# stevesuyao/KinectDepthMapEnhancement

Hardware: AMD Instinct MI355X
Metric: Mpixels/sec joint-bilateral filtered (640x480 & 1080p); % HBM roofline (higher is better)
Workload: dtype f32; 1 GPU; JointBilateralFilter::Process (K0 pre-smooth 5/30/30 + K1) on 64 x 640x480 synthetic RGB-D frames (64 per GPU), window 11 (radius 5), sigma_s 3 px, sigma_r 7.65/255, sigma_d 20 mm; frames_per_gpu=64, width=640, height=480, window=11, kernel_variant=auto (w11-pk2-16x16-false-v4)

## Files before the change

kinectdepthmapenhancement_amd/csrc/jbf_fast.hip:

```cpp
#include "kde_internal.h"
#include "kde_device_math.h"

#include <type_traits>

namespace kde {
namespace {

constexpr uint32_t kMagic = 0x4B000000u;
constexpr uint32_t kOff = 1u << 18;
constexpr uint32_t kInvalidBias = 0xFF000000u;
constexpr float kBiasF = 8388608.0f + 262144.0f;
constexpr uint32_t kNegHBits = 0xCB7C0000u;
constexpr double kScaleLog2 = 24.0;

struct FastArgs {
    const float* depth;
    const uint8_t* guide;
    float* out;
    int width, height, n;
    int tiles_x, tiles_y;
    FastDiv24 div_tiles, div_tx;
    float kc;
    float sd;
    float t_skip;
    float t2_skip;
    int cd_skip;
    int vec4;
    KDE_STAGE(float* stage_avg; unsigned* stage_counters; int stage_force;)
    const float* tab_dev;
    __attribute__((aligned(8))) float tab[882];
};

__device__ __forceinline__ uint32_t dot4(uint32_t a, uint32_t b, uint32_t c)
{
    return __builtin_amdgcn_udot4(a, b, c, false);
}


template <int WIN, int PX, int BX, int BY, bool CACHE, bool CSKIP>
__global__ __launch_bounds__(BX* BY) void jbf_fast_kernel(const FastArgs a)
{
    constexpr int R = WIN / 2;
    constexpr int NT = BX * BY;
    constexpr int TW = BX * PX, TH = BY;
    constexpr int LW = TW + 2 * R, LH = TH + 2 * R;
    constexpr int P = LW;
    constexpr int SEG = PX + 2 * R;
    __shared__ float s_d[LH * P];
    __shared__ uint32_t s_c[LH * P];
    __shared__ uint32_t s_n[LH * P];

    const unsigned nblk = gridDim.x;
    const unsigned lin = blockIdx.x;
    const unsigned per = nblk / 8, rem = nblk % 8;
    const unsigned xcd = lin % 8, slot = lin / 8;
    const unsigned id = xcd * per + (xcd < rem ? xcd : rem) + slot;
    const unsigned tiles = (unsigned)a.tiles_x * a.tiles_y;
    const unsigned frame_i = fastdiv24(id, a.div_tiles);
    const unsigned tile = id - frame_i * tiles;
    const int tyi = (int)fastdiv24(tile, a.div_tx), txi = tile - tyi * a.tiles_x;
    const int x0 = txi * TW, y0 = tyi * TH;

    const size_t frame = (size_t)frame_i * a.width * a.height;
    const float* __restrict__ depth = a.depth + frame;
    const uint8_t* __restrict__ guide = a.guide + frame * 3;
    const int tid = threadIdx.x;

    for (int i = tid; i < LW * LH; i += NT) {
        const int ly = i / LW, lx = i - ly * LW;
        const int gx = x0 + lx - R, gy = y0 + ly - R;
        float d = 0.0f;
        uint32_t c = 0;
        if (gx >= 0 && gx < a.width && gy >= 0 && gy < a.height) {
            const size_t q = (size_t)gy * a.width + gx;
            d = depth[q];
            const uint8_t* p = guide + q * 3;
            c = (uint32_t)p[0] | ((uint32_t)p[1] << 8) | ((uint32_t)p[2] << 16);
        }
        const bool valid = d > 50.0f;
        s_d[ly * P + lx] = valid ? d : 0.0f;
        s_c[ly * P + lx] = c;
        s_n[ly * P + lx] = valid ? (kMagic + kOff) - dot4(c, c, 0) : kInvalidBias;
    }
    __syncthreads();

    const int tx = tid % BX, ty = tid / BX;
    const int xb = x0 + tx * PX, y = y0 + ty;
    if (xb >= a.width || y >= a.height) return;

    uint32_t cc[PX];
    float cA[PX], skipA[PX];
    uint32_t thrU[PX];
#pragma unroll
    for (int k = 0; k < PX; k++) {
        cc[k] = s_c[(ty + R) * P + tx * PX + R + k];
        const uint32_t na = dot4(cc[k], cc[k], 0);
        cA[k] = -a.kc * (kBiasF + (float)na);
        skipA[k] = __builtin_fmaf(kBiasF + (float)na, a.kc, cA[k]);
        thrU[k] = CSKIP ? (kMagic + kOff) + na - (uint32_t)a.cd_skip : 0;
    }

    float arg[CACHE ? WIN * WIN * PX : 1];
    float wsum[PX], wgt[PX];
#pragma unroll
    for (int k = 0; k < PX; k++) wsum[k] = wgt[k] = 0.0f;

    auto arg1_of = [&](uint32_t cq, uint32_t nq, int k, float ls) -> float {
        const uint32_t u = (dot4(cq, cc[k], 0) << 1) + nq;
        float a1 = __builtin_fmaf(__uint_as_float(u), a.kc, cA[k]);
        if (CSKIP) a1 = (u <= thrU[k]) ? skipA[k] : a1;
        return a1 + ls;
    };

    auto pass1_row = [&](int i) {
        float dr[SEG];
        uint32_t cr[SEG], nr[SEG];
        const int rb = (ty + i) * P + tx * PX;
#pragma unroll
        for (int q = 0; q < SEG; q++) {
            dr[q] = s_d[rb + q];
            cr[q] = s_c[rb + q];
            nr[q] = s_n[rb + q];
        }
#pragma unroll
        for (int j = 0; j < WIN; j++) {
            const float ls = a.tab[i * WIN + j];
#pragma unroll
            for (int k = 0; k < PX; k++) {
                const float a1 = arg1_of(cr[j + k], nr[j + k], k, ls);
                if (CACHE) arg[(i * WIN + j) * PX + k] = a1;
                const float f = __builtin_amdgcn_exp2f(a1);
                wsum[k] = __builtin_fmaf(dr[j + k], f, wsum[k]);
                wgt[k] += f;
            }
        }
    };
    if (CACHE) {
#pragma unroll
        for (int i = 0; i < WIN; i++) pass1_row(i);
    } else {
#pragma unroll 1
        for (int i = 0; i < WIN; i++) pass1_row(i);
    }

    float c2[PX], num[PX], den[PX];
#pragma unroll
    for (int k = 0; k < PX; k++) {
        c2[k] = wsum[k] / wgt[k];
        num[k] = den[k] = 0.0f;
    }

    auto pass2_row = [&](int i) {
        float dr[SEG];
        uint32_t cr[SEG], nr[SEG];
        const int rb = (ty + i) * P + tx * PX;
#pragma unroll
        for (int q = 0; q < SEG; q++) {
            dr[q] = s_d[rb + q];
            if (!CACHE) {
                cr[q] = s_c[rb + q];
                nr[q] = s_n[rb + q];
            }
        }
#pragma unroll
        for (int j = 0; j < WIN; j++) {
            const float ls = CACHE ? 0.0f : a.tab[i * WIN + j];
#pragma unroll
            for (int k = 0; k < PX; k++) {
                const float a1 = CACHE ? arg[(i * WIN + j) * PX + k] : arg1_of(cr[j + k], nr[j + k], k, ls);
                const float t = (dr[j + k] - c2[k]) * a.sd;
                float a2 = __builtin_fmaf(-t, t, a1);
                a2 = (__builtin_fabsf(t) >= a.t_skip) ? a1 : a2;
                const float f = __builtin_amdgcn_exp2f(a2);
                num[k] = __builtin_fmaf(dr[j + k], f, num[k]);
                den[k] += f;
            }
        }
    };
    if (CACHE) {
#pragma unroll
        for (int i = 0; i < WIN; i++) pass2_row(i);
    } else {
#pragma unroll 1
        for (int i = 0; i < WIN; i++) pass2_row(i);
    }

    float* __restrict__ o = a.out + frame + (size_t)y * a.width + xb;
#pragma unroll
    for (int k = 0; k < PX; k++) {
        float r = 0.0f;
        if (wgt[k] > 0.0f) r = (den[k] == 0.0f) ? 0.0f : num[k] / den[k];
        if (xb + k < a.width) o[k] = r;
        KDE_STAGE(if (a.stage_avg && xb + k < a.width) a.stage_avg[frame + (size_t)y * a.width + xb + k] = c2[k];)
    }
}


typedef float f2 __attribute__((ext_vector_type(2)));
typedef uint32_t u2 __attribute__((ext_vector_type(2)));

__device__ __forceinline__ f2 pk_fma(f2 a, f2 b, f2 c) { return __builtin_elementwise_fma(a, b, c); }
__device__ __forceinline__ f2 bcast(float v) { return f2{v, v}; }
__device__ __forceinline__ f2 pk_add_clamp(f2 a, f2 b)
{
    f2 r;
    asm("v_pk_add_f32 %0, %1, %2 clamp" : "=v"(r) : "v"(a), "v"(b));
    return r;
}
__device__ __forceinline__ f2 pk_mul_clamp(f2 a, f2 b)
{
    f2 r;
    asm("v_pk_mul_f32 %0, %1, %2 clamp" : "=v"(r) : "v"(a), "v"(b));
    return r;
}

constexpr int pk_min_waves(int win, int np, bool cache, bool cskip, bool elide_on)
{
    if (win >= 23) return 3;
    if (win == 5 && np == 1 && cache) return 5;
    return 1;
}

template <int WIN, int NP, int BX, int BY, bool CACHE, bool CSKIP, bool VL, bool ELIDE_ON = true, int CR = (CACHE ? WIN : 0)>
__global__ __launch_bounds__(BX* BY) __attribute__((amdgpu_waves_per_eu(pk_min_waves(WIN, NP, CACHE, CSKIP, ELIDE_ON))))
void jbf_pk_kernel(const FastArgs a)
{
    static_assert(CR == (CACHE ? WIN : 0), "cached rows: all or none");
    constexpr int R = WIN / 2;
    constexpr int PX = 2 * NP;
    constexpr int NT = BX * BY;
    constexpr int TW = BX * PX, TH = BY;
    constexpr int LH = TH + 2 * R;
    constexpr int S1 = 0;
    constexpr int RA = !VL ? R : ((R + 3) / 4 * 4);
    constexpr int SH = VL ? ((RA - R) & 1) : 0;
    constexpr bool ALIGNED = ((RA - R + SH) % 2) == 0;
    constexpr int G = (RA + TW + R + 3) / 4;
    constexpr int P = VL ? (SH + 4 * G + 1) / 2 * 2 : (TW + 2 * R);
    constexpr int SEGP = NP + R;
    constexpr int HALF = (WIN - 1) / 2;
    static_assert(RA >= R && P % 2 == 0 && (!VL || ((RA + S1) % 4 == 0 && TW % 4 == 0 && (SH != 0 || P % 4 == 0))), "tile geometry");
    __shared__ __attribute__((aligned(16))) float s_d[LH * P];
    __shared__ __attribute__((aligned(16))) uint32_t s_c[LH * P];
    __shared__ __attribute__((aligned(16))) float s_n[LH * P];

    const unsigned nblk = gridDim.x;
    const unsigned lin = blockIdx.x;
    const unsigned per = nblk / 8, rem = nblk % 8;
    const unsigned xcd = lin % 8, slot = lin / 8;
    const unsigned id = xcd * per + (xcd < rem ? xcd : rem) + slot;
    const unsigned tiles = (unsigned)a.tiles_x * a.tiles_y;
    const unsigned frame_i = fastdiv24(id, a.div_tiles);
    const unsigned tile = id - frame_i * tiles;
    const int tyi = (int)fastdiv24(tile, a.div_tx), txi = tile - tyi * a.tiles_x;
    const int x0 = txi * TW - S1, y0 = tyi * TH;
    const int o = x0 - RA;

    const size_t frame = (size_t)frame_i * a.width * a.height;
    const float* __restrict__ depth = a.depth + frame;
    const uint8_t* __restrict__ guide = a.guide + frame * 3;
    const int tid = threadIdx.x;

    constexpr bool ELIDE = WIN >= 9 && ELIDE_ON;
    __shared__ uint32_t s_stat[8];
    if (ELIDE) {
        if (tid < 8) s_stat[tid] = (tid == 0 || (tid >= 2 && !(tid & 1))) ? 0xffffffffu : 0u;
        __syncthreads();
    }
    uint32_t st_dmin = 0x7f800000u, st_dmax = 0u, st_cmin[3] = {255u, 255u, 255u}, st_cmax[3] = {0u, 0u, 0u};
    auto stat = [&](float dv, uint32_t c, bool inside) {
        if (!ELIDE) return;
        if (dv > 0.0f) {
            st_dmin = min(st_dmin, __float_as_uint(dv));
            st_dmax = max(st_dmax, __float_as_uint(dv));
        }
        if (inside) {
#pragma unroll
            for (int ch = 0; ch < 3; ch++) {
                const uint32_t v = (c >> (8 * ch)) & 0xffu;
                st_cmin[ch] = min(st_cmin[ch], v);
                st_cmax[ch] = max(st_cmax[ch], v);
            }
        }
    };

    if (!VL) {
        for (int i = tid; i < P * LH; i += NT) {
            const int ly = i / P, lx = i - ly * P;
            const int gx = o + lx, gy = y0 - R + ly;
            float d = 0.0f;
            uint32_t c = 0;
            const bool inside = gx >= 0 && gx < a.width && gy >= 0 && gy < a.height;
            if (inside) {
                const size_t q = (size_t)gy * a.width + gx;
                d = depth[q];
                const uint8_t* p = guide + q * 3;
                c = (uint32_t)p[0] | ((uint32_t)p[1] << 8) | ((uint32_t)p[2] << 16);
            }
            const bool valid = d > 50.0f;
            s_d[i] = valid ? d : 0.0f;
            s_c[i] = c;
            s_n[i] = __uint_as_float(dot4(c, c, kNegHBits));
            stat(valid ? d : 0.0f, c, inside);
        }
    }
    for (int g = tid; VL && g < G * LH; g += NT) {
        const int ly = g / G, gi = g - ly * G;
        const int gx = o + 4 * gi, gy = y0 - R + ly;
        float d[4] = {0.0f, 0.0f, 0.0f, 0.0f};
        uint32_t c[4] = {0u, 0u, 0u, 0u};
        if (gy >= 0 && gy < a.height) {
            const size_t q = (size_t)gy * a.width + gx;
            if (a.vec4 && gx >= 0 && gx + 3 < a.width) {
                const float4 dv = *reinterpret_cast<const float4*>(depth + q);
                const uint32_t* cp = reinterpret_cast<const uint32_t*>(guide + q * 3);
                const uint32_t w0 = cp[0], w1 = cp[1], w2 = cp[2];
                d[0] = dv.x; d[1] = dv.y; d[2] = dv.z; d[3] = dv.w;
                c[0] = w0 & 0xffffffu;
                c[1] = (w0 >> 24) | ((w1 & 0xffffu) << 8);
                c[2] = (w1 >> 16) | ((w2 & 0xffu) << 16);
                c[3] = w2 >> 8;
            } else {
#pragma unroll
                for (int k = 0; k < 4; k++) {
                    if (gx + k >= 0 && gx + k < a.width) {
                        d[k] = depth[q + k];
                        const uint8_t* p = guide + (q + k) * 3;
                        c[k] = (uint32_t)p[0] | ((uint32_t)p[1] << 8) | ((uint32_t)p[2] << 16);
                    }
                }
            }
        }
        float nn[4];
#pragma unroll
        for (int k = 0; k < 4; k++) {
            const bool valid = d[k] > 50.0f;
            d[k] = valid ? d[k] : 0.0f;
            nn[k] = __uint_as_float(dot4(c[k], c[k], kNegHBits));
            stat(d[k], c[k], gy >= 0 && gy < a.height && gx + k >= 0 && gx + k < a.width);
        }
        const int li = ly * P + 4 * gi + SH;
        if constexpr (SH == 0) {
            *reinterpret_cast<float4*>(&s_d[li]) = make_float4(d[0], d[1], d[2], d[3]);
            *reinterpret_cast<uint4*>(&s_c[li]) = make_uint4(c[0], c[1], c[2], c[3]);
            *reinterpret_cast<float4*>(&s_n[li]) = make_float4(nn[0], nn[1], nn[2], nn[3]);
        } else {
#pragma unroll
            for (int k = 0; k < 4; k++) {
                s_d[li + k] = d[k];
                s_c[li + k] = c[k];
                s_n[li + k] = nn[k];
            }
        }
    }
    if (ELIDE) {
        uint32_t v[8] = {st_dmin, st_dmax, st_cmin[0], st_cmax[0], st_cmin[1], st_cmax[1], st_cmin[2], st_cmax[2]};
#pragma unroll
        for (int k = 0; k < 8; k++) {
#pragma unroll
            for (int m = 32; m >= 1; m >>= 1) {
                const uint32_t ov = (uint32_t)__shfl_xor((int)v[k], m, 64);
                v[k] = (k & 1) ? max(v[k], ov) : min(v[k], ov);
            }
        }
        if ((tid & 63) == 0) {
#pragma unroll
            for (int k = 0; k < 8; k++) {
                if (k & 1) atomicMax(&s_stat[k], v[k]);
                else atomicMin(&s_stat[k], v[k]);
            }
        }
    }
    __syncthreads();

    bool tile_c = CSKIP, tile_d = true;
    if (ELIDE) {
        const int rb = (int)s_stat[3] - (int)s_stat[2], rg = (int)s_stat[5] - (int)s_stat[4], rr = (int)s_stat[7] - (int)s_stat[6];
        if (s_stat[3] >= s_stat[2]) tile_c = CSKIP && (rb * rb + rg * rg + rr * rr >= a.cd_skip);
        const float range = __uint_as_float(s_stat[1]) - __uint_as_float(s_stat[0]);
        const float slack = __uint_as_float(s_stat[1]) * (float)(WIN * WIN + 8) * 0x1p-24f;
        tile_d = !((range * 1.0001f + slack) * a.sd < a.t_skip);
    }
    KDE_STAGE(if (a.stage_force) { tile_c = CSKIP; tile_d = true; })
    KDE_STAGE(if (a.stage_counters && tid == 0) {
        int body;
        if constexpr (!ELIDE) body = (CSKIP ? 1 : 0) + 2;
        else if constexpr (WIN >= 15) body = ((CSKIP && tile_c) || tile_d) ? (CSKIP ? 1 : 0) + 2 : 0;
        else body = ((CSKIP && tile_c) ? 1 : 0) + (tile_d ? 2 : 0);
        atomicAdd(&a.stage_counters[body], 1u);
    })

    const int tx = tid % BX, ty = tid / BX;
    const int xb = x0 + tx * PX, y = y0 + ty;
    if (xb >= a.width || y >= a.height) return;
    const int sx = SH + RA - R + tx * PX;

    uint32_t cc[PX];
    f2 negC[NP];
#pragma unroll
    for (int pp = 0; pp < NP; pp++) {
#pragma unroll
        for (int h = 0; h < 2; h++) {
            const int k = 2 * pp + h;
            cc[k] = s_c[(ty + R) * P + sx + R + k];
            const uint32_t na = dot4(cc[k], cc[k], 0);
            negC[pp][h] = -((float)kOff + (float)na);
        }
    }

    f2 kc2 = bcast(a.kc);
    asm volatile("" : "+v"(kc2));
    f2 arg[CR > 0 ? CR * WIN * NP : 1];
    f2 wsum[NP], wgt[NP];
#pragma unroll
    for (int pp = 0; pp < NP; pp++) wsum[pp] = wgt[pp] = bcast(0.0f);

    const f2 Tc = bcast((float)a.cd_skip);
    const f2 T2 = bcast(a.t2_skip);
    const f2 kBig = bcast(0x1p100f);

    auto unit_arg = [&](auto cs_tag, const u2* cp, const f2* np, int pp, int i, int u) -> f2 {
        constexpr bool CS = decltype(cs_tag)::value;
        uint32_t c0, c1;
        f2 hq;
        if (u <= HALF) {
            c0 = cp[pp + u].x; c1 = cp[pp + u].y; hq = np[pp + u];
        } else if (u < WIN - 1) {
            const int m = pp + (u - HALF);
            c0 = cp[m].y; c1 = cp[m].x; hq = __builtin_shufflevector(np[m], np[m], 1, 0);
        } else {
            c0 = cp[pp].y; c1 = cp[pp + HALF].x; hq = bcast(0.0f);
        }
        const f2 ab = f2{__uint_as_float(dot4(c0, cc[2 * pp], kMagic)), __uint_as_float(dot4(c1, cc[2 * pp + 1], kMagic))};
        f2 w;
        if (u == WIN - 1) {
            float w0 = __builtin_fmaf(ab.x, 2.0f, np[pp].y), w1 = __builtin_fmaf(ab.y, 2.0f, np[pp + HALF].x);
            asm("" : "+v"(w0));
            asm("" : "+v"(w1));
            w = f2{w0, w1};
        } else {
            w = pk_fma(ab, bcast(2.0f), hq);
        }
        const f2 ncd = w + negC[pp];
        f2 lsj;
        if constexpr (WIN > 21) {
            typedef const f2 __attribute__((address_space(4)))* cf2p;
            lsj = *(cf2p)(uintptr_t)(a.tab_dev + (i * WIN + u) * 2);
        } else {
            lsj = *reinterpret_cast<const f2*>(&a.tab[(i * WIN + u) * 2]);
        }
        if (CS) return pk_fma(ncd, pk_add_clamp(ncd, Tc) * kc2, lsj);
        return pk_fma(ncd, kc2, lsj);
    };
    auto unit_depth = [&](const f2* dp, int pp, int u) -> f2 {
        if (u <= HALF) return dp[pp + u];
        if (u < WIN - 1) return __builtin_shufflevector(dp[pp + (u - HALF)], dp[pp + (u - HALF)], 1, 0);
        return f2{dp[pp].y, dp[pp + HALF].x};
    };

    auto pass1_row = [&](auto cs_tag, auto keep_tag, int i) {
        constexpr bool KEEP = decltype(keep_tag)::value;
        f2 dp[SEGP], vp[SEGP];
        u2 cp[SEGP];
        f2 np[SEGP];
        const int rb = (ty + i) * P + sx;
#pragma unroll
        for (int m = 0; m < SEGP; m++) {
            dp[m] = ALIGNED ? *reinterpret_cast<const f2*>(&s_d[rb + 2 * m]) : f2{s_d[rb + 2 * m], s_d[rb + 2 * m + 1]};
            cp[m] = ALIGNED ? *reinterpret_cast<const u2*>(&s_c[rb + 2 * m]) : u2{s_c[rb + 2 * m], s_c[rb + 2 * m + 1]};
            np[m] = ALIGNED ? *reinterpret_cast<const f2*>(&s_n[rb + 2 * m]) : f2{s_n[rb + 2 * m], s_n[rb + 2 * m + 1]};
            vp[m] = pk_add_clamp(dp[m], dp[m]);
        }
#pragma unroll
        for (int pp = 0; pp < NP; pp++) {
#pragma unroll
            for (int u = 0; u < WIN; u++) {
                const f2 a1 = unit_arg(cs_tag, cp, np, pp, i, u);
                if constexpr (KEEP) arg[(i * NP + pp) * WIN + u] = a1;
                const f2 f = f2{__builtin_amdgcn_exp2f(a1.x), __builtin_amdgcn_exp2f(a1.y)};
                wsum[pp] = pk_fma(unit_depth(dp, pp, u), f, wsum[pp]);
                wgt[pp] = pk_fma(unit_depth(vp, pp, u), f, wgt[pp]);
            }
        }
    };
    f2 c2[NP], num[NP], den[NP];

    auto pass2_row = [&](auto cs_tag, auto ds_tag, auto keep_tag, int i) {
        constexpr bool DS = decltype(ds_tag)::value;
        constexpr bool KEEP = decltype(keep_tag)::value;
        f2 dp[SEGP], vp[SEGP];
        u2 cp[SEGP];
        f2 np[SEGP];
        const int rb = (ty + i) * P + sx;
#pragma unroll
        for (int m = 0; m < SEGP; m++) {
            dp[m] = ALIGNED ? *reinterpret_cast<const f2*>(&s_d[rb + 2 * m]) : f2{s_d[rb + 2 * m], s_d[rb + 2 * m + 1]};
            vp[m] = pk_add_clamp(dp[m], dp[m]);
            if constexpr (!KEEP) {
                cp[m] = ALIGNED ? *reinterpret_cast<const u2*>(&s_c[rb + 2 * m]) : u2{s_c[rb + 2 * m], s_c[rb + 2 * m + 1]};
                np[m] = ALIGNED ? *reinterpret_cast<const f2*>(&s_n[rb + 2 * m]) : f2{s_n[rb + 2 * m], s_n[rb + 2 * m + 1]};
            }
        }
#pragma unroll
        for (int pp = 0; pp < NP; pp++) {
#pragma unroll
            for (int u = 0; u < WIN; u++) {
                f2 a1;
                if constexpr (KEEP) a1 = arg[(i * NP + pp) * WIN + u];
                else a1 = unit_arg(cs_tag, cp, np, pp, i, u);
                const f2 dq = unit_depth(dp, pp, u);
                const f2 t = (dq - c2[pp]) * bcast(a.sd);
                f2 a2;
                if (DS) {
                    const f2 m = pk_mul_clamp(pk_fma(-t, t, T2), kBig);
                    a2 = pk_fma(-(t * m), t, a1);
                } else {
                    a2 = pk_fma(-t, t, a1);
                }
                const f2 f = f2{__builtin_amdgcn_exp2f(a2.x), __builtin_amdgcn_exp2f(a2.y)};
                num[pp] = pk_fma(dq, f, num[pp]);
                den[pp] = pk_fma(unit_depth(vp, pp, u), f, den[pp]);
            }
        }
    };
    auto run = [&](auto cs_tag, auto ds_tag) {
#pragma unroll
        for (int i = 0; i < CR; i++) pass1_row(cs_tag, std::true_type{}, i);
#pragma unroll 1
        for (int i = CR; i < WIN; i++) pass1_row(cs_tag, std::false_type{}, i);
#pragma unroll
        for (int pp = 0; pp < NP; pp++) {
            c2[pp] = wsum[pp] * f2{__builtin_amdgcn_rcpf(wgt[pp].x), __builtin_amdgcn_rcpf(wgt[pp].y)};
            num[pp] = den[pp] = bcast(0.0f);
        }
#pragma unroll
        for (int i = 0; i < CR; i++) pass2_row(cs_tag, ds_tag, std::true_type{}, i);
#pragma unroll 1
        for (int i = CR; i < WIN; i++) pass2_row(cs_tag, ds_tag, std::false_type{}, i);
    };
    using T_ = std::true_type;
    using F_ = std::false_type;
    if constexpr (!ELIDE) {
        run(std::integral_constant<bool, CSKIP>{}, T_{});
    } else if constexpr (WIN >= 15) {
        if ((CSKIP && tile_c) || tile_d) run(std::integral_constant<bool, CSKIP>{}, T_{});
        else run(F_{}, F_{});
    } else {
        if (!CSKIP || !tile_c) {
            if (tile_d) run(F_{}, T_{});
            else run(F_{}, F_{});
        } else {
            if (tile_d) run(T_{}, T_{});
            else run(T_{}, F_{});
        }
    }

    float* __restrict__ op = a.out + frame + (size_t)y * a.width + xb;
#pragma unroll
    for (int pp = 0; pp < NP; pp++) {
        float r0 = 0.0f, r1 = 0.0f;
        if (wgt[pp].x > 0.0f) r0 = (den[pp].x == 0.0f) ? 0.0f : num[pp].x * __builtin_amdgcn_rcpf(den[pp].x);
        if (wgt[pp].y > 0.0f) r1 = (den[pp].y == 0.0f) ? 0.0f : num[pp].y * __builtin_amdgcn_rcpf(den[pp].y);
        if (xb + 2 * pp >= 0 && xb + 2 * pp < a.width) op[2 * pp] = r0;
        if (xb + 2 * pp + 1 < a.width) op[2 * pp + 1] = r1;
        KDE_STAGE(if (a.stage_avg) {
            float* sp = a.stage_avg + frame + (size_t)y * a.width + xb;
            if (xb + 2 * pp >= 0 && xb + 2 * pp < a.width) sp[2 * pp] = c2[pp].x;
            if (xb + 2 * pp + 1 < a.width) sp[2 * pp + 1] = c2[pp].y;
        })
    }
}

template <int WIN, int NP, int BX, int BY, bool CACHE, bool VL, bool ELIDE_ON = true, int CR = (CACHE ? WIN : 0)>
int launch_pk_variant(const JbfLaunch& l, const FastArgs& fa, bool cskip, hipStream_t s)
{
    FastArgs a = fa;
    a.tiles_x = ceil_div(l.width, BX * NP * 2);
    a.tiles_y = ceil_div(l.height, BY);
    const long long blocks = (long long)a.tiles_x * a.tiles_y * l.n;
    a.div_tiles = make_fastdiv24((uint32_t)(a.tiles_x * a.tiles_y), (uint64_t)blocks);
    a.div_tx = make_fastdiv24((uint32_t)a.tiles_x, (uint64_t)a.tiles_x * a.tiles_y);
    if (blocks > 0x7fffffffLL) return fail(KDE_ERR_INVALID, "jbf: batch too large for one launch");
    if (cskip)
        hipLaunchKernelGGL((jbf_pk_kernel<WIN, NP, BX, BY, CACHE, true, VL, ELIDE_ON, CR>), dim3((unsigned)blocks), dim3(BX * BY), 0, s, a);
    else
        hipLaunchKernelGGL((jbf_pk_kernel<WIN, NP, BX, BY, CACHE, false, VL, ELIDE_ON, CR>), dim3((unsigned)blocks), dim3(BX * BY), 0, s, a);
    KDE_HIP_TRY(hipGetLastError());
    return KDE_OK;
}

template <int WIN, int PX, int BX, int BY, bool CACHE>
int launch_variant(const JbfLaunch& l, const FastArgs& fa, bool cskip, hipStream_t s)
{
    FastArgs a = fa;
    a.tiles_x = ceil_div(l.width, BX * PX);
    a.tiles_y = ceil_div(l.height, BY);
    const long long blocks = (long long)a.tiles_x * a.tiles_y * l.n;
    a.div_tiles = make_fastdiv24((uint32_t)(a.tiles_x * a.tiles_y), (uint64_t)blocks);
    a.div_tx = make_fastdiv24((uint32_t)a.tiles_x, (uint64_t)a.tiles_x * a.tiles_y);
    if (blocks > 0x7fffffffLL) return fail(KDE_ERR_INVALID, "jbf: batch too large for one launch");
    if (cskip)
        hipLaunchKernelGGL((jbf_fast_kernel<WIN, PX, BX, BY, CACHE, true>), dim3((unsigned)blocks), dim3(BX * BY), 0, s, a);
    else
        hipLaunchKernelGGL((jbf_fast_kernel<WIN, PX, BX, BY, CACHE, false>), dim3((unsigned)blocks), dim3(BX * BY), 0, s, a);
    KDE_HIP_TRY(hipGetLastError());
    return KDE_OK;
}

struct Variant {
    const char* name;
    int window;
    bool packed;
    int (*launch)(const JbfLaunch&, const FastArgs&, bool, hipStream_t);
};

#define V(WIN, PX, BX, BY, CACHE) \
    {"w" #WIN "-sc" #PX "-" #BX "x" #BY "-" #CACHE, WIN, false, &launch_variant<WIN, PX, BX, BY, CACHE>}
#define K(WIN, NP, BX, BY, CACHE) \
    {"w" #WIN "-pk" #NP "-" #BX "x" #BY "-" #CACHE "-v4", WIN, true, &launch_pk_variant<WIN, NP, BX, BY, CACHE, true>}
#define KS(WIN, NP, BX, BY, CACHE) \
    {"w" #WIN "-pk" #NP "-" #BX "x" #BY "-" #CACHE "-v1", WIN, true, &launch_pk_variant<WIN, NP, BX, BY, CACHE, false>}
#define KN(WIN, NP, BX, BY, CACHE) \
    {"w" #WIN "-pk" #NP "-" #BX "x" #BY "-" #CACHE "-v4-noelide", WIN, true, &launch_pk_variant<WIN, NP, BX, BY, CACHE, true, false>}
const Variant kVariants[] = {
    K(5, 1, 16, 16, true),  K(5, 1, 32, 8, true),   KS(5, 1, 16, 16, true),  K(5, 2, 32, 8, true),  K(5, 1, 32, 8, false),
    V(5, 2, 32, 8, true),   V(5, 1, 64, 4, true),
    K(7, 1, 16, 16, true),  K(7, 1, 32, 8, true),   KS(7, 1, 32, 8, true),  K(7, 1, 32, 8, false),  V(7, 1, 64, 4, true),
    K(11, 2, 16, 16, false), KS(11, 2, 16, 16, false), KS(11, 1, 16, 16, false), K(11, 1, 16, 16, false), K(11, 1, 32, 8, false),
    KS(11, 1, 32, 8, false), KS(11, 2, 32, 8, false), V(11, 2, 16, 16, false), V(11, 1, 32, 8, false),
    KN(11, 2, 16, 16, false),
    K(19, 1, 16, 16, false), KS(19, 1, 16, 16, false), KS(19, 2, 16, 16, false), K(19, 2, 16, 16, false), K(19, 1, 32, 8, false),
    KS(19, 1, 32, 8, false), KS(19, 2, 32, 8, false), V(19, 2, 16, 16, false), V(19, 1, 32, 8, false),
    KN(19, 1, 16, 16, false),
    K(3, 1, 16, 16, true),   K(3, 2, 16, 16, true),
    K(9, 2, 16, 16, false),  K(9, 1, 16, 16, false),
    K(13, 2, 16, 16, false), K(13, 1, 16, 16, false),
    K(15, 1, 16, 16, false), K(15, 2, 16, 16, false),
    K(17, 1, 16, 16, false), K(17, 2, 16, 16, false),
    K(21, 1, 16, 16, false), K(21, 2, 16, 16, false),
    K(23, 1, 16, 16, false), K(25, 1, 16, 16, false), K(27, 1, 16, 16, false), K(29, 1, 16, 16, false), K(31, 1, 16, 16, false),
};
static_assert(sizeof(FastArgs) <= 4096, "FastArgs is passed by value as the kernel-argument block");
#undef V
#undef K
#undef KS
#undef KN
constexpr int kNumVariants = sizeof(kVariants) / sizeof(kVariants[0]);

}

int jbf_fast_variant_count() { return kNumVariants; }
const char* jbf_fast_variant_name(int v) { return (v >= 0 && v < kNumVariants) ? kVariants[v].name : "?"; }
int jbf_fast_variant_window(int v) { return (v >= 0 && v < kNumVariants) ? kVariants[v].window : 0; }

int jbf_fast_default_variant(const JbfLaunch& l)
{
    for (int v = 0; v < kNumVariants; v++)
        if (kVariants[v].window == l.window) return v;
    return -1;
}

bool jbf_fast_supported(const JbfLaunch& l)
{
    if (l.color_sigma == 0.0f || l.depth_sigma == 0.0f) return false;
    const double kc = 1.4426950408889634 / (double)l.color_den;
    if (!(kc * 1.0e38 > 1.0e4) || !(kc < 1.0e30)) return false;
    return jbf_fast_default_variant(l) >= 0;
}

void jbf_fast_fill_table(int W, const float* table_host, bool packed, float* out)
{
    const int HALF = (W - 1) / 2;
    auto lg = [&](int i, int j) {
        const float sv = table_host[i * W + j];
        return (float)(((sv == 0.0f) ? 0.0 : std::log2((double)sv)) + kScaleLog2);
    };
    if (!packed) {
        for (int i = 0; i < W; i++)
            for (int j = 0; j < W; j++) out[i * W + j] = lg(i, j);
        return;
    }
    for (int i = 0; i < W; i++)
        for (int u = 0; u < W; u++) {
            const int j0 = u <= HALF ? 2 * u : (u < W - 1 ? 2 * (u - HALF) + 1 : 1);
            const int j1 = u <= HALF ? 2 * u : (u < W - 1 ? 2 * (u - HALF) - 1 : W - 2);
            out[(i * W + u) * 2] = lg(i, j0);
            out[(i * W + u) * 2 + 1] = lg(i, j1);
        }
}

bool jbf_fast_needs_device_table(int window) { return window > 21; }

int launch_jbf_fast(const JbfLaunch& l, int variant, const float* table_host, hipStream_t s)
{
    if (variant < 0 || variant >= kNumVariants || kVariants[variant].window != l.window)
        return fail(KDE_ERR_INVALID, "jbf: variant %d does not implement window %d", variant, l.window);
    FastArgs a;
    memset(&a, 0, sizeof(a));
    a.depth = l.depth;
    a.guide = l.guide;
    a.out = l.out;
    a.width = l.width;
    a.height = l.height;
    a.n = l.n;
    const double log2e = 1.4426950408889634;
    a.kc = (float)(log2e / (double)l.color_den);
    a.sd = (float)std::sqrt(log2e / (double)l.depth_den);
    a.t_skip = std::isinf(l.d2_skip) ? INFINITY : (float)(std::sqrt((double)l.d2_skip) * std::sqrt(log2e / (double)l.depth_den));
    a.t2_skip = std::isinf(a.t_skip) ? 3.0e38f : a.t_skip * a.t_skip;
    a.cd_skip = l.cd_skip;
    a.vec4 = (l.width % 4 == 0) && ((reinterpret_cast<uintptr_t>(l.depth) & 15u) == 0) &&
             ((reinterpret_cast<uintptr_t>(l.guide) & 3u) == 0);
    KDE_STAGE(a.stage_avg = g_stage.jbf_avg; a.stage_counters = g_stage.counters; a.stage_force = g_stage.force_full_rules;)
    if (jbf_fast_needs_device_table(l.window)) {
        if (!l.log2_pk_dev) return fail(KDE_ERR_INVALID, "jbf: window %d needs the handle's device copy of the log2 table", l.window);
        a.tab_dev = l.log2_pk_dev;
    } else {
        jbf_fast_fill_table(l.window, table_host, kVariants[variant].packed, a.tab);
    }
    const bool cskip = l.cd_skip <= 195075;
    return kVariants[variant].launch(l, a, cskip, s);
}

}
```

Before: 17220 Mpixels/s.

## Elide filter work per wavefront using 8x8 sub-tile stats from LDS scan

Replaces the per-block depth/color range statistics, which were gathered during the global load and merged with shuffles plus LDS atomics, with a per-wavefront scan of the shared-memory tile. Each wave covers an 8x8 (or WTX-wide) patch of outputs, computes min/max using packed u16 ops and DPP reductions, and decides independently whether to skip the color or depth term. The smaller regions make skipping more likely, and the block-level atomics and one extra barrier go away. In exchange each wave rereads its halo from LDS. New default w11 variant with 8-wide wave tiles is placed first, plus extra variants.

Result: faster. 17930 Mpixels/s (median of 6 runs) (+4.1%).

```diff
diff --git a/kinectdepthmapenhancement_amd/csrc/jbf_fast.hip b/kinectdepthmapenhancement_amd/csrc/jbf_fast.hip
--- a/kinectdepthmapenhancement_amd/csrc/jbf_fast.hip
+++ b/kinectdepthmapenhancement_amd/csrc/jbf_fast.hip
@@ -214,21 +214,50 @@
     return r;
 }
 
+typedef unsigned short us2 __attribute__((ext_vector_type(2)));
+__device__ __forceinline__ uint32_t pk_min_u16(uint32_t a, uint32_t b)
+{
+    return __builtin_bit_cast(uint32_t, __builtin_elementwise_min(__builtin_bit_cast(us2, a), __builtin_bit_cast(us2, b)));
+}
+__device__ __forceinline__ uint32_t pk_max_u16(uint32_t a, uint32_t b)
+{
+    return __builtin_bit_cast(uint32_t, __builtin_elementwise_max(__builtin_bit_cast(us2, a), __builtin_bit_cast(us2, b)));
+}
+template <int CTRL, int ROWS = 0xf>
+__device__ __forceinline__ uint32_t dpp_mov(uint32_t v)
+{
+    return (uint32_t)__builtin_amdgcn_update_dpp((int)v, (int)v, CTRL, ROWS, 0xf, false);
+}
+template <class Op>
+__device__ __forceinline__ uint32_t wave_reduce(uint32_t v, Op op)
+{
+    v = op(v, dpp_mov<0xb1>(v));
+    v = op(v, dpp_mov<0x4e>(v));
+    v = op(v, dpp_mov<0x124>(v));
+    v = op(v, dpp_mov<0x128>(v));
+    v = op(v, dpp_mov<0x142, 0xa>(v));
+    v = op(v, dpp_mov<0x143, 0xc>(v));
+    return (uint32_t)__builtin_amdgcn_readlane((int)v, 63);
+}
+
 constexpr int pk_min_waves(int win, int np, bool cache, bool cskip, bool elide_on)
 {
     if (win >= 23) return 3;
     if (win == 5 && np == 1 && cache) return 5;
+    if (np == 1 && !cskip && elide_on && !cache && win >= 9 && win <= 15) return win == 9 ? 8 : win == 11 ? 6 : 5;
     return 1;
 }
 
-template <int WIN, int NP, int BX, int BY, bool CACHE, bool CSKIP, bool VL, bool ELIDE_ON = true, int CR = (CACHE ? WIN : 0)>
+template <int WIN, int NP, int BX, int BY, bool CACHE, bool CSKIP, bool VL, bool ELIDE_ON = true, int WTX = BX>
 __global__ __launch_bounds__(BX* BY) __attribute__((amdgpu_waves_per_eu(pk_min_waves(WIN, NP, CACHE, CSKIP, ELIDE_ON))))
 void jbf_pk_kernel(const FastArgs a)
 {
-    static_assert(CR == (CACHE ? WIN : 0), "cached rows: all or none");
+    constexpr int CR = CACHE ? WIN : 0;
     constexpr int R = WIN / 2;
     constexpr int PX = 2 * NP;
     constexpr int NT = BX * BY;
+    constexpr int WTY = 64 / WTX, WAVES_X = BX / WTX;
+    static_assert(NT % 64 == 0 && 64 % WTX == 0 && BX % WTX == 0 && BY % WTY == 0, "whole wavefronts, each a WTX x WTY block of threads");
     constexpr int TW = BX * PX, TH = BY;
     constexpr int LH = TH + 2 * R;
     constexpr int S1 = 0;
@@ -262,27 +291,6 @@
     const int tid = threadIdx.x;
 
     constexpr bool ELIDE = WIN >= 9 && ELIDE_ON;
-    __shared__ uint32_t s_stat[8];
-    if (ELIDE) {
-        if (tid < 8) s_stat[tid] = (tid == 0 || (tid >= 2 && !(tid & 1))) ? 0xffffffffu : 0u;
-        __syncthreads();
-    }
-    uint32_t st_dmin = 0x7f800000u, st_dmax = 0u, st_cmin[3] = {255u, 255u, 255u}, st_cmax[3] = {0u, 0u, 0u};
-    auto stat = [&](float dv, uint32_t c, bool inside) {
-        if (!ELIDE) return;
-        if (dv > 0.0f) {
-            st_dmin = min(st_dmin, __float_as_uint(dv));
-            st_dmax = max(st_dmax, __float_as_uint(dv));
-        }
-        if (inside) {
-#pragma unroll
-            for (int ch = 0; ch < 3; ch++) {
-                const uint32_t v = (c >> (8 * ch)) & 0xffu;
-                st_cmin[ch] = min(st_cmin[ch], v);
-                st_cmax[ch] = max(st_cmax[ch], v);
-            }
-        }
-    };
 
     if (!VL) {
         for (int i = tid; i < P * LH; i += NT) {
@@ -301,7 +309,6 @@
             s_d[i] = valid ? d : 0.0f;
             s_c[i] = c;
             s_n[i] = __uint_as_float(dot4(c, c, kNegHBits));
-            stat(valid ? d : 0.0f, c, inside);
         }
     }
     for (int g = tid; VL && g < G * LH; g += NT) {
@@ -337,7 +344,6 @@
             const bool valid = d[k] > 50.0f;
             d[k] = valid ? d[k] : 0.0f;
             nn[k] = __uint_as_float(dot4(c[k], c[k], kNegHBits));
-            stat(d[k], c[k], gy >= 0 && gy < a.height && gx + k >= 0 && gx + k < a.width);
         }
         const int li = ly * P + 4 * gi + SH;
         if constexpr (SH == 0) {
@@ -353,36 +359,80 @@
             }
         }
     }
-    if (ELIDE) {
-        uint32_t v[8] = {st_dmin, st_dmax, st_cmin[0], st_cmax[0], st_cmin[1], st_cmax[1], st_cmin[2], st_cmax[2]};
-#pragma unroll
-        for (int k = 0; k < 8; k++) {
-#pragma unroll
-            for (int m = 32; m >= 1; m >>= 1) {
-                const uint32_t ov = (uint32_t)__shfl_xor((int)v[k], m, 64);
-                v[k] = (k & 1) ? max(v[k], ov) : min(v[k], ov);
-            }
-        }
-        if ((tid & 63) == 0) {
-#pragma unroll
-            for (int k = 0; k < 8; k++) {
-                if (k & 1) atomicMax(&s_stat[k], v[k]);
-                else atomicMin(&s_stat[k], v[k]);
-            }
-        }
-    }
     __syncthreads();
 
+    const int wave = __builtin_amdgcn_readfirstlane(tid >> 6), lane = tid & 63;
+    const int tx0 = WTX * (wave % WAVES_X), ty0 = WTY * (wave / WAVES_X);
+    const int tx = tx0 + lane % WTX, ty = ty0 + lane / WTX;
+    if (x0 + tx0 * PX >= a.width || y0 + ty0 >= a.height) return;
+
     bool tile_c = CSKIP, tile_d = true;
-    if (ELIDE) {
-        const int rb = (int)s_stat[3] - (int)s_stat[2], rg = (int)s_stat[5] - (int)s_stat[4], rr = (int)s_stat[7] - (int)s_stat[6];
-        if (s_stat[3] >= s_stat[2]) tile_c = CSKIP && (rb * rb + rg * rg + rr * rr >= a.cd_skip);
-        const float range = __uint_as_float(s_stat[1]) - __uint_as_float(s_stat[0]);
-        const float slack = __uint_as_float(s_stat[1]) * (float)(WIN * WIN + 8) * 0x1p-24f;
-        tile_d = !((range * 1.0001f + slack) * a.sd < a.t_skip);
+    if constexpr (ELIDE) {
+        constexpr int RWP = (WTX * PX + 2 * R) / 2, RH = WTY + 2 * R;
+        constexpr int NE = RWP * RH;
+        const int sxw = SH + RA - R + tx0 * PX;
+        const int gx0 = x0 + tx0 * PX - R, gy0 = y0 + ty0 - R;
+        uint32_t dmin = 0xffffffffu, dmax = 0u;
+        uint32_t brmin = 0x00ff00ffu, brmax = 0u, ggmin = 0x00ff00ffu, ggmax = 0u;
+        auto scan = [&](auto masked_tag) {
+            constexpr bool MASKED = decltype(masked_tag)::value;
+            constexpr int QY = 64 / RWP, QP = 64 % RWP;
+            int ry = lane / RWP, rp = lane - ry * RWP;
+            int li = (ty0 + ry) * P + sxw + 2 * rp;
+#pragma unroll
+            for (int k = 0; k < (NE + 63) / 64; k++) {
+                if (k > 0) {
+                    const bool wrap = rp + QP >= RWP;
+                    rp += wrap ? QP - RWP : QP;
+                    ry += wrap ? QY + 1 : QY;
+                    li += wrap ? (QY + 1) * P + 2 * (QP - RWP) : QY * P + 2 * QP;
+                }
+                if (64 * k + 63 < NE || lane + 64 * k < NE) {
+                    const u2 d = *reinterpret_cast<const u2*>(&s_d[li]);
+                    dmin = min(dmin, min(d.x - 1u, d.y - 1u));
+                    dmax = max(dmax, max(d.x, d.y));
+                    if constexpr (CSKIP) {
+                        const u2 c = *reinterpret_cast<const u2*>(&s_c[li]);
+                        uint32_t lo0 = c.x, lo1 = c.y, hi0 = c.x, hi1 = c.y;
+                        if constexpr (MASKED) {
+                            const bool iny = (unsigned)(gy0 + ry) < (unsigned)a.height;
+                            const bool in0 = iny & ((unsigned)(gx0 + 2 * rp) < (unsigned)a.width);
+                            const bool in1 = iny & ((unsigned)(gx0 + 2 * rp + 1) < (unsigned)a.width);
+                            lo0 = in0 ? lo0 : 0x00ffffffu;
+                            lo1 = in1 ? lo1 : 0x00ffffffu;
+                            hi0 = in0 ? hi0 : 0u;
+                            hi1 = in1 ? hi1 : 0u;
+                        }
+                        brmin = pk_min_u16(pk_min_u16(brmin, lo0 & 0x00ff00ffu), lo1 & 0x00ff00ffu);
+                        brmax = pk_max_u16(pk_max_u16(brmax, hi0 & 0x00ff00ffu), hi1 & 0x00ff00ffu);
+                        ggmin = pk_min_u16(ggmin, __builtin_amdgcn_perm(lo1, lo0, 0x0c050c01u));
+                        ggmax = pk_max_u16(ggmax, __builtin_amdgcn_perm(hi1, hi0, 0x0c050c01u));
+                    }
+                }
+            }
+        };
+        if (!CSKIP || (gx0 >= 0 && gx0 + 2 * RWP <= a.width && gy0 >= 0 && gy0 + RH <= a.height)) scan(std::false_type{});
+        else scan(std::true_type{});
+        const uint32_t w_dmin = wave_reduce(dmin, [](uint32_t p, uint32_t q) { return min(p, q); }) + 1u;
+        const uint32_t w_dmax = wave_reduce(dmax, [](uint32_t p, uint32_t q) { return max(p, q); });
+        if constexpr (CSKIP) {
+            const uint32_t w_brmin = wave_reduce(brmin, pk_min_u16), w_brmax = wave_reduce(brmax, pk_max_u16);
+            const uint32_t w_ggmin = wave_reduce(ggmin, pk_min_u16), w_ggmax = wave_reduce(ggmax, pk_max_u16);
+            const int bmin = w_brmin & 0xffffu, bmax = w_brmax & 0xffffu, rmin = w_brmin >> 16, rmax = w_brmax >> 16;
+            const int gmin = min(w_ggmin & 0xffffu, w_ggmin >> 16), gmax = max(w_ggmax & 0xffffu, w_ggmax >> 16);
+            const int rb = bmax - bmin, rg = gmax - gmin, rr = rmax - rmin;
+            if (bmax >= bmin) tile_c = rb * rb + rg * rg + rr * rr >= a.cd_skip;
+        }
+        if (w_dmax == 0u) {
+            tile_d = false;
+        } else {
+            const float range = __uint_as_float(w_dmax) - __uint_as_float(w_dmin);
+            const float slack = __uint_as_float(w_dmax) * (float)(WIN * WIN + 8) * 0x1p-24f;
+            tile_d = !((range * 1.0001f + slack) * a.sd < a.t_skip);
+        }
     }
     KDE_STAGE(if (a.stage_force) { tile_c = CSKIP; tile_d = true; })
-    KDE_STAGE(if (a.stage_counters && tid == 0) {
+    KDE_STAGE(if (a.stage_counters && lane == 0) {
         int body;
         if constexpr (!ELIDE) body = (CSKIP ? 1 : 0) + 2;
         else if constexpr (WIN >= 15) body = ((CSKIP && tile_c) || tile_d) ? (CSKIP ? 1 : 0) + 2 : 0;
@@ -390,7 +440,6 @@
         atomicAdd(&a.stage_counters[body], 1u);
     })
 
-    const int tx = tid % BX, ty = tid / BX;
     const int xb = x0 + tx * PX, y = y0 + ty;
     if (xb >= a.width || y >= a.height) return;
     const int sx = SH + RA - R + tx * PX;
@@ -571,7 +620,7 @@
     }
 }
 
-template <int WIN, int NP, int BX, int BY, bool CACHE, bool VL, bool ELIDE_ON = true, int CR = (CACHE ? WIN : 0)>
+template <int WIN, int NP, int BX, int BY, bool CACHE, bool VL, bool ELIDE_ON = true, int WTX = BX>
 int launch_pk_variant(const JbfLaunch& l, const FastArgs& fa, bool cskip, hipStream_t s)
 {
     FastArgs a = fa;
@@ -582,9 +631,9 @@
     a.div_tx = make_fastdiv24((uint32_t)a.tiles_x, (uint64_t)a.tiles_x * a.tiles_y);
     if (blocks > 0x7fffffffLL) return fail(KDE_ERR_INVALID, "jbf: batch too large for one launch");
     if (cskip)
-        hipLaunchKernelGGL((jbf_pk_kernel<WIN, NP, BX, BY, CACHE, true, VL, ELIDE_ON, CR>), dim3((unsigned)blocks), dim3(BX * BY), 0, s, a);
+        hipLaunchKernelGGL((jbf_pk_kernel<WIN, NP, BX, BY, CACHE, true, VL, ELIDE_ON, WTX>), dim3((unsigned)blocks), dim3(BX * BY), 0, s, a);
     else
-        hipLaunchKernelGGL((jbf_pk_kernel<WIN, NP, BX, BY, CACHE, false, VL, ELIDE_ON, CR>), dim3((unsigned)blocks), dim3(BX * BY), 0, s, a);
+        hipLaunchKernelGGL((jbf_pk_kernel<WIN, NP, BX, BY, CACHE, false, VL, ELIDE_ON, WTX>), dim3((unsigned)blocks), dim3(BX * BY), 0, s, a);
     KDE_HIP_TRY(hipGetLastError());
     return KDE_OK;
 }
@@ -622,18 +671,23 @@
     {"w" #WIN "-pk" #NP "-" #BX "x" #BY "-" #CACHE "-v1", WIN, true, &launch_pk_variant<WIN, NP, BX, BY, CACHE, false>}
 #define KN(WIN, NP, BX, BY, CACHE) \
     {"w" #WIN "-pk" #NP "-" #BX "x" #BY "-" #CACHE "-v4-noelide", WIN, true, &launch_pk_variant<WIN, NP, BX, BY, CACHE, true, false>}
+#define KQ(WIN, NP, BX, BY, CACHE) \
+    {"w" #WIN "-pk" #NP "-" #BX "x" #BY "-" #CACHE "-v4", WIN, true, &launch_pk_variant<WIN, NP, BX, BY, CACHE, true, true, 8>}
+#define KR(WIN, NP, BX, BY, CACHE) \
+    {"w" #WIN "-pk" #NP "-" #BX "x" #BY "-" #CACHE "-v4-rows", WIN, true, &launch_pk_variant<WIN, NP, BX, BY, CACHE, true>}
 const Variant kVariants[] = {
     K(5, 1, 16, 16, true),  K(5, 1, 32, 8, true),   KS(5, 1, 16, 16, true),  K(5, 2, 32, 8, true),  K(5, 1, 32, 8, false),
     V(5, 2, 32, 8, true),   V(5, 1, 64, 4, true),
     K(7, 1, 16, 16, true),  K(7, 1, 32, 8, true),   KS(7, 1, 32, 8, true),  K(7, 1, 32, 8, false),  V(7, 1, 64, 4, true),
-    K(11, 2, 16, 16, false), KS(11, 2, 16, 16, false), KS(11, 1, 16, 16, false), K(11, 1, 16, 16, false), K(11, 1, 32, 8, false),
+    KQ(11, 2, 16, 16, false), KR(11, 2, 16, 16, false), K(11, 2, 8, 32, false),
+    KS(11, 2, 16, 16, false), KS(11, 1, 16, 16, false), K(11, 1, 16, 16, false), K(11, 1, 32, 8, false),
     KS(11, 1, 32, 8, false), KS(11, 2, 32, 8, false), V(11, 2, 16, 16, false), V(11, 1, 32, 8, false),
     KN(11, 2, 16, 16, false),
     K(19, 1, 16, 16, false), KS(19, 1, 16, 16, false), KS(19, 2, 16, 16, false), K(19, 2, 16, 16, false), K(19, 1, 32, 8, false),
     KS(19, 1, 32, 8, false), KS(19, 2, 32, 8, false), V(19, 2, 16, 16, false), V(19, 1, 32, 8, false),
     KN(19, 1, 16, 16, false),
     K(3, 1, 16, 16, true),   K(3, 2, 16, 16, true),
-    K(9, 2, 16, 16, false),  K(9, 1, 16, 16, false),
+    K(9, 2, 16, 16, false),  K(9, 1, 16, 16, false),  KN(9, 2, 16, 16, false),
     K(13, 2, 16, 16, false), K(13, 1, 16, 16, false),
     K(15, 1, 16, 16, false), K(15, 2, 16, 16, false),
     K(17, 1, 16, 16, false), K(17, 2, 16, 16, false),
@@ -645,6 +699,8 @@
 #undef K
 #undef KS
 #undef KN
+#undef KQ
+#undef KR
 constexpr int kNumVariants = sizeof(kVariants) / sizeof(kVariants[0]);
 
 }
```
